# menickname/waafle

Hardware: AMD Instinct MI355X
Metric: contigs scored/sec + k2 clade-pair evals/sec at 1/2/4/8 MI355X vs CPU ref (higher is better)
Workload: dtype f64

## Files before the change

### waafle_amd/csrc/wf_device.h

```cpp
#pragma once
#include "wf_internal.h"

#include "waafle_hip.h"
#include "wf_lanes.h"

namespace wf {

namespace {


constexpr uint64_t kKeyPad = ~0ull;

#include "wf_stamps.h"
constexpr int kLocVirtual = 0xFFFF;

__device__ __forceinline__ void note_ppot(const KArgs& K, int c, int iteration, int Pp) {
  if (!K.ppot || Pp < 2) return;
  const uint64_t old = (uint64_t)K.ppot[c];
  if (iteration > (int)(old >> 40))
    K.ppot[c] = (int64_t)(((uint64_t)iteration << 40) | ((old & ((1ull << 40) - 1ull)) + (uint64_t)Pp));
}

__device__ __forceinline__ bool e2_no_option(const KArgs& K, int c, int iteration, int64_t pair_evals, bool root,
                                             int32_t* pend) {
// ... 90 lines not shown
    int a = __shfl_up(x, d, 64), b = __shfl_up(y, d, 64);
    if (lane >= d) { x += a; y += b; }
  }
  if (lane == 63) { ctl.red_i[w] = x; ctl.red_j[w] = y; }
  __syncthreads();
  int b1 = 0, b2 = 0, s1 = 0, s2 = 0;
#pragma unroll
  for (int i = 0; i < NT / 64; ++i) {
    int a = ctl.red_i[i], b = ctl.red_j[i];
    if (i < w) { b1 += a; b2 += b; }
    s1 += a;
    s2 += b;
  }
  __syncthreads();
  *p1 = b1 + x - v1;
  *p2 = b2 + y - v2;
  *t1 = s1;
  *t2 = s2;
}

__device__ __forceinline__ bool better(double r2, long long k2, double r, long long k) {
  return k2 >= 0 && (k < 0 || r2 > r || (r2 == r && k2 > k));
}

template <int NT>
__device__ __forceinline__ void block_argmax(double& r, long long& k, Ctl& ctl) {
#pragma unroll
  for (int off = 32; off > 0; off >>= 1) {
    double r2 = __shfl_xor(r, off, 64);
    long long k2 = __shfl_xor(k, off, 64);
    if (better(r2, k2, r, k)) { r = r2; k = k2; }
  }
  if (lane_id() == 0) { ctl.red_r[wave_id()] = r; ctl.red_k[wave_id()] = k; }
  __syncthreads();
  if (threadIdx.x == 0) {
    double br = ctl.red_r[0];
    long long bk = ctl.red_k[0];
    for (int i = 1; i < NT / 64; ++i)
      if (better(ctl.red_r[i], ctl.red_k[i], br, bk)) { br = ctl.red_r[i]; bk = ctl.red_k[i]; }
    ctl.best_r = br;
    ctl.best_k = bk;
  }
  __syncthreads();
  r = ctl.best_r;
  k = ctl.best_k;
}

template <int NT, class T>
__device__ __forceinline__ void bitonic_sort(T* keys, int n) {
  for (int k = 2; k <= n; k <<= 1) {
    for (int j = k >> 1; j > 0; j >>= 1) {
      for (int i = threadIdx.x; i < n; i += NT) {
        int ixj = i ^ j;
        if (ixj > i) {
          T a = keys[i], b = keys[ixj];
          bool up = (i & k) == 0;
          if ((a > b) == up) { keys[i] = b; keys[ixj] = a; }
        }
      }
      __syncthreads();
    }
  }
}


__device__ __forceinline__ int lca2(const KArgs& K, int a, int b) {
  if (a < 0) return b;
  if (b < 0) return a;
  if (a == b) return a;
  if (K.lin) {
    const int4* ra = reinterpret_cast<const int4*>(K.lin + (int64_t)a * kLin);
    const int4* rb = reinterpret_cast<const int4*>(K.lin + (int64_t)b * kLin);
    int4 x[kLin / 4], y[kLin / 4];
#pragma unroll
    for (int i = 0; i < kLin / 4; ++i) { x[i] = ra[i]; y[i] = rb[i]; }
    int r = x[0].x;
#pragma unroll
    for (int i = 0; i < kLin / 4; ++i) {
      if (x[i].x >= 0 && x[i].x == y[i].x) r = x[i].x;
      if (x[i].y >= 0 && x[i].y == y[i].y) r = x[i].y;
      if (x[i].z >= 0 && x[i].z == y[i].z) r = x[i].z;
      if (x[i].w >= 0 && x[i].w == y[i].w) r = x[i].w;
    }
    return r;
  }
  int da = K.depth[a], db = K.depth[b];
  while (da > db) { a = K.parent[a]; --da; }
  while (db > da) { b = K.parent[b]; --db; }
  while (a != b) { a = K.parent[a]; b = K.parent[b]; }
  return a;
}

__device__ __forceinline__ int block_lca(const KArgs& K, const int* list, int m, Ctl& ctl) {
  if (m <= 0) return -1;
  if (m == 1) return list[0];
  if (wave_id() == 0) {
    int acc = -1;
    for (int i = lane_id(); i < m; i += 64) acc = lca2(K, acc, list[i]);
#pragma unroll
    for (int off = 32; off > 0; off >>= 1) {
      int o = __shfl_xor(acc, off, 64);
      acc = lca2(K, acc, o);
    }
    if (lane_id() == 0) ctl.lca_out = acc;
  }
  __syncthreads();
  int r = ctl.lca_out;
  __syncthreads();
  return r;
}


constexpr int kMaxDepth = 7;
constexpr int kGroupMax = 64;

__device__ int gen_leaves(int off0, int cl, int4* out, int8_t* sched = nullptr, int stride = 0) {
  int so[8], sl[8], ss[8], sf[8];
#pragma unroll
  for (int i = 0; i < 8; ++i) { so[i] = 0; sl[i] = 0; ss[i] = 0; sf[i] = 0; }
  int cnt = 0;
  auto push = [&](int o, int l) {
#pragma unroll
    for (int i = 7; i > 0; --i) { so[i] = so[i - 1]; sl[i] = sl[i - 1]; ss[i] = ss[i - 1]; sf[i] = sf[i - 1]; }
    so[0] = o; sl[0] = l; ss[0] = 0; sf[0] = cnt;
  };
  auto pop = [&]() {
#pragma unroll
    for (int i = 0; i < 7; ++i) { so[i] = so[i + 1]; sl[i] = sl[i + 1]; ss[i] = ss[i + 1]; sf[i] = sf[i + 1]; }
  };
  int sp = 1;
  so[0] = off0; sl[0] = cl; ss[0] = 0; sf[0] = 0;
  while (sp > 0) {
    if (sl[0] > kLeafMax && ss[0] == 0) {
      int h = sl[0] / 2;
      h -= h % 8;
      ss[0] = 1;
      push(so[0], h);
      ++sp;
      continue;
    }
    const int lo = so[0], ll = sl[0];
    int adds = 0;
    pop();
    --sp;
    ++cnt;
    while (sp > 0) {
      if (ss[0] == 1) {
        int h = sl[0] / 2;
        h -= h % 8;
        ss[0] = 2;
        if (sched && sp - 1 < kMaxDepth && sf[0] < stride)
          sched[sf[0] * 8 + (sp - 1)] = (int8_t)cnt;
        push(so[0] + h, sl[0] - h);
        ++sp;
        break;
      }
      ++adds;
      pop();
      --sp;
    }
    if (out) out[cnt - 1] = make_int4(lo, ll, adds, 0);
  }
  return cnt;
}

__device__ int leaves_of_length(int n) {
  int cnt = 0;
  for (int o = 0; o < n; o += kNpyBuf) cnt += gen_leaves(o, min(kNpyBuf, n - o), nullptr);
  return cnt;
}

template <class F>
__device__ double serial_block(int o, int l, F f) {
  if (l < 8) {
    double r = 0.0;
    for (int i = 0; i < l; ++i) r += f(o + i);
    return r;
  }
  double r0 = f(o), r1 = f(o + 1), r2 = f(o + 2), r3 = f(o + 3);
  double r4 = f(o + 4), r5 = f(o + 5), r6 = f(o + 6), r7 = f(o + 7);
  int i = 8;
  const int m = l - (l & 7);
  for (; i < m; i += 8) {
    r0 += f(o + i); r1 += f(o + i + 1); r2 += f(o + i + 2); r3 += f(o + i + 3);
    r4 += f(o + i + 4); r5 += f(o + i + 5); r6 += f(o + i + 6); r7 += f(o + i + 7);
  }
  double res = ((r0 + r1) + (r2 + r3)) + ((r4 + r5) + (r6 + r7));
  for (; i < l; ++i) res += f(o + i);
  return res;
}

template <class F>
__device__ double serial_pairwise(int off0, int cl, F f) {
  if (cl <= kLeafMax) return serial_block(off0, cl, f);
  int so[8], sl[8], ss[8];
#pragma unroll
  for (int i = 0; i < 8; ++i) { so[i] = 0; sl[i] = 0; ss[i] = 0; }
  auto push = [&](int o, int l) {
#pragma unroll
    for (int i = 7; i > 0; --i) { so[i] = so[i - 1]; sl[i] = sl[i - 1]; ss[i] = ss[i - 1]; }
    so[0] = o; sl[0] = l; ss[0] = 0;
  };
  auto pop = [&]() {
#pragma unroll
    for (int i = 0; i < 7; ++i) { so[i] = so[i + 1]; sl[i] = sl[i + 1]; ss[i] = ss[i + 1]; }
  };
  double a0 = 0.0, a1 = 0.0, a2 = 0.0, a3 = 0.0, a4 = 0.0, a5 = 0.0, a6 = 0.0, a7 = 0.0;
  int sp = 1;
  so[0] = off0; sl[0] = cl;
  while (sp > 0) {
    if (sl[0] > kLeafMax && ss[0] == 0) {
      int h = sl[0] / 2;
      h -= h % 8;
      ss[0] = 1;
      push(so[0], h);
      ++sp;
      continue;
    }
    const double v = serial_block(so[0], sl[0], f);
    a7 = a6; a6 = a5; a5 = a4; a4 = a3; a3 = a2; a2 = a1; a1 = a0; a0 = v;
    pop();
    --sp;
    while (sp > 0) {
      if (ss[0] == 1) {
        int h = sl[0] / 2;
        h -= h % 8;
        ss[0] = 2;
        push(so[0] + h, sl[0] - h);
        ++sp;
        break;
      }
      a0 = a1 + a0;
      a1 = a2; a2 = a3; a3 = a4; a4 = a5; a5 = a6; a6 = a7;
      pop();
      --sp;
    }
  }
  return a0;
}

template <class F>
__device__ __forceinline__ double np_sum(int n, F f) {
  if (n <= kLeafMax) return 0.0 + serial_block(0, n, f);
  double total = 0.0;
  for (int o = 0; o < n; o += kNpyBuf) total += serial_pairwise(o, min(kNpyBuf, n - o), f);
  return total;
}


struct Contig {
  int64_t h0, l0, mbase;
  int H, G;
  int *loc_lo, *loc_len, *loc_st, *leaf_off;
  int *loc_grp, *loc_steps, *sched_off;
  uint64_t* sched;
  int4* leaves;
  int *alo, *ahi, *ahit, *aloc, *acl;
  double* asc;
  uint64_t* maxes;
  int *ign, *um;
  uint64_t* keys;
  int *seg_start, *seg_cl, *cl_id, *pot, *mem1, *mem2, *sorder;
  double* S;
  uint64_t* mask;
  unsigned *bm1, *bm2;
  uint8_t* best_syn;
  char* xws = nullptr;
  int64_t xcap = 0;
  int* sib_of = nullptr;
  uint64_t* hm = nullptr;
};

struct SumStack {
  double s0 = 0.0, s1 = 0.0, s2 = 0.0, s3 = 0.0, s4 = 0.0, s5 = 0.0, s6 = 0.0, s7 = 0.0;
  __device__ __forceinline__ void push(double v) {
    s7 = s6; s6 = s5; s5 = s4; s4 = s3; s3 = s2; s2 = s1; s1 = s0; s0 = v;
  }
  __device__ __forceinline__ void add_top() {
    s0 = s1 + s0;
    s1 = s2; s2 = s3; s3 = s4; s4 = s5; s5 = s6; s6 = s7;
  }
};

__device__ __forceinline__ double seqsum(double v, int cnt) {
  double r = 0.0;
  for (int i = 0; i < cnt; ++i) r += v;
  return r;
}

__device__ __forceinline__ double leaf_tree(double r0, double r1, double r2, double r3, double r4,
                                            double r5, double r6, double r7) {
  return ((r0 + r1) + (r2 + r3)) + ((r4 + r5) + (r6 + r7));
}

__device__ __forceinline__ int below(int base, int bound, int m) {
  const int d = bound - base;
  return d <= 0 ? 0 : min(m, (d + 7) >> 3);
}

constexpr int kThreadLeaves = 32;
constexpr int kE2Seg = 320;
constexpr int kE2MaxG = 63;
constexpr int kPruneMax = 64;

__device__ __forceinline__ bool attaches(const DevParams& P, int qlo, int qhi, int hs, int l1,
                                         int len, int lst) {
  if (P.stranded && hs != lst) return false;
  const int l2 = l1 + len - 1;
  if (l1 > qhi || qlo > l2) return 0.0 >= P.min_overlap;
  const int ov = min(qhi, l2) - max(qlo, l1) + 1;
  const int den = min(qhi - qlo + 1, l2 - l1 + 1);
  if (ov == den) return 1.0 >= P.min_overlap;
  const double t = (double)den * P.min_overlap;
  if ((double)ov > t + fabs(t) * 1e-9) return true;
  if ((double)ov < t - fabs(t) * 1e-9) return false;
  return (double)ov / (double)den >= P.min_overlap;
}

__device__ __forceinline__ double run_leaf(int lo, int hi, double v, int st, int ln) {
  const int m = ln >> 3, be = st + (m << 3);
  hi = max(hi, lo);
  double res = 0.0;
  if (m > 0) {
    int k[8], kmin = m;
#pragma unroll
    for (int c = 0; c < 8; ++c) {
      k[c] = below(st + c, hi, m) - below(st + c, lo, m);
      kmin = min(kmin, k[c]);
    }
    double s0 = 0.0;
    for (int i = 0; i < kmin; ++i) s0 += v;
    const double s1 = s0 + v, s2 = s1 + v;
    double r[8];
#pragma unroll
    for (int c = 0; c < 8; ++c) r[c] = k[c] == kmin ? s0 : (k[c] == kmin + 1 ? s1 : s2);
    res = leaf_tree(r[0], r[1], r[2], r[3], r[4], r[5], r[6], r[7]);
  }
  for (int x = be; x < st + ln; ++x) res += (x >= lo && x < hi) ? v : 0.0;
  return res;
}

template <class F>
__device__ __forceinline__ double np_sum_seq(int n, F next) {
  if (n < 8) {
    double r = 0.0;
    for (int i = 0; i < n; ++i) r += next();
    return r;
  }
  double r0 = next(), r1 = next(), r2 = next(), r3 = next();
  double r4 = next(), r5 = next(), r6 = next(), r7 = next();
  int i = 8;
  const int m = n - (n & 7);
  for (; i < m; i += 8) {
    r0 += next(); r1 += next(); r2 += next(); r3 += next();
    r4 += next(); r5 += next(); r6 += next(); r7 += next();
  }
  double res = ((r0 + r1) + (r2 + r3)) + ((r4 + r5) + (r6 + r7));
  for (; i < n; ++i) res += next();
  return res;
}

struct PtrLut {
  const int4* p;
  __device__ __forceinline__ int4 operator()(int q) const { return p[q]; }
};
__device__ __forceinline__ uint32_t pack_leaf(int4 e) { return (uint32_t)e.x | ((uint32_t)e.y << 13) | ((uint32_t)e.z << 21); }
struct PackedLut {
  const uint32_t* p;
  __device__ __forceinline__ int4 operator()(int q) const {
    const uint32_t u = p[q];
    return make_int4((int)(u & 8191u), (int)((u >> 13) & 255u), (int)(u >> 21), 0);
  }
};

__device__ __forceinline__ double pw_const_sum(int n, double v) {
  const int a0 = n >> 4;
  int K = 0, m = n;
  unsigned sel = 0;
  while (m > 128) {
    const int a = m >> 4;
    sel |= (a != (a0 >> K) ? 1u : 0u) << K;
    m -= 8 * a;
    ++K;
  }
  int Db = 0, Dmax = -1, xB = 0, xC = 0;
  bool need16 = false;
  if (K > 0) {
    Db = max(0, 28 - __clz(a0));
    Dmax = max(K - 1, Db);
    xB = a0 >> Db;
    xC = Dmax == Db + 1 ? a0 >> (Db + 1) : 0;
    need16 = Db >= 1 && (a0 >> (Db - 1)) == 16;
  }
  const int mL = m < 8 ? m : m >> 3;
  const int imax = max(max(xB, mL), need16 ? 16 : 0);
  double t = 0.0, sB = 0.0, sC = 0.0, sL = 0.0;
  for (int i = 1; i <= imax; ++i) {
    t += v;
    sB = i == xB ? t : sB;
    sC = i == xC ? t : sC;
    sL = i == mL ? t : sL;
  }
  double R;
  if (m < 8) {
    R = sL;
  } else {
    R = 8.0 * sL;
    for (int x = 0; x < (m & 7); ++x) R += v;
  }
  double q0 = 0.0, q1 = 0.0;
  for (int d = Dmax; d >= 0; --d) {
    const int B = a0 >> d;
    if (d >= Db) {
      const double sd = d == Db ? sB : sC;
      q0 = 8.0 * sd;
      q1 = 8.0 * (sd + v);
    } else {
      const double c0 = q0, c1 = q1;
      q0 = (B & 1) ? c0 + c1 : c0 + c0;
      q1 = (B & 1) ? c1 + c1 : c0 + c1;
      if (B == 16) q0 = 8.0 * t;
    }
    if (d < K) R = (((sel >> d) & 1u) ? q1 : q0) + R;
  }
  return R;
}

struct LeafCode { int kmin, code; };
__device__ __forceinline__ LeafCode run_leaf_code(int lo, int hi, int st, int ln) {
  const int m = ln >> 3, be = st + (m << 3);
  hi = max(hi, lo);
  int k[8], kmin = m;
#pragma unroll
  for (int c = 0; c < 8; ++c) {
    k[c] = below(st + c, hi, m) - below(st + c, lo, m);
    kmin = min(kmin, k[c]);
  }
  int code = 0;
#pragma unroll
  for (int c = 0; c < 8; ++c) code |= min(k[c] - kmin, 2) << (2 * c);
  const int tail = max(0, min(st + ln, hi) - max(be, lo));
  return LeafCode{kmin, code | (tail << 16) | (m > 0 ? 1 << 20 : 0)};
}
__device__ __forceinline__ double run_leaf_value(double v, LeafCode lc, double s0) {
  double res = 0.0;
  if ((lc.code >> 20) & 1) {
    const double s1 = s0 + v, s2 = s1 + v;
    double r[8];
#pragma unroll
    for (int c = 0; c < 8; ++c) {
      const int d = (lc.code >> (2 * c)) & 3;
      r[c] = d == 0 ? s0 : (d == 1 ? s1 : s2);
    }
    res = leaf_tree(r[0], r[1], r[2], r[3], r[4], r[5], r[6], r[7]);
  }
  for (int x = (lc.code >> 16) & 15; x > 0; --x) res += v;
  return res;
}

__device__ __forceinline__ double pw_run_sum(int n, int lo, int hi, double v) {
  lo = max(lo, 0);
  hi = min(hi, n);
  if (hi <= lo) return 0.0;
  const int a0 = n >> 4;
  int K = 0, m = n;
  unsigned sel = 0;
  while (m > 128) {
    const int a = m >> 4;
    sel |= (a != (a0 >> K) ? 1u : 0u) << K;
    m -= 8 * a;
    ++K;
  }
  int Db = 0, Dmax = -1, xB = 0, xC = 0;
  bool need16 = false;
  if (K > 0) {
    Db = max(0, 28 - __clz(a0));
    Dmax = max(K - 1, Db);
    xB = a0 >> Db;
    xC = Dmax == Db + 1 ? a0 >> (Db + 1) : 0;
    need16 = Db >= 1 && (a0 >> (Db - 1)) == 16;
  }
  struct Nd { int s, z, kind, cls, t; };
  auto child = [&](const Nd& x, bool right) -> Nd {
    if (x.kind == 0) {
      const int nl = 8 * (x.z >> 4);
      return right ? Nd{x.s + nl, x.z - nl, 0, 0, x.t + 1} : Nd{x.s, nl, 1, (int)((sel >> x.t) & 1u), x.t + 1};
    }
    const int xx = x.z >> 3, xl = xx >> 1, Bt = a0 >> x.t;
    return right ? Nd{x.s + 8 * xl, 8 * (xx - xl), 1, (xx - xl) - Bt, x.t + 1} : Nd{x.s, 8 * xl, 1, xl - Bt, x.t + 1};
  };
  Nd nd{0, n, 0, 0, 0};
  int mode = 0;
  for (;;) {
    if (lo <= nd.s && hi >= nd.s + nd.z) { mode = 1; break; }
    if (nd.z <= 128) { mode = 2; break; }
    const int nl = nd.kind == 0 ? 8 * (nd.z >> 4) : 8 * ((nd.z >> 3) >> 1);
    if (hi <= nd.s + nl) nd = child(nd, false);
    else if (lo >= nd.s + nl) nd = child(nd, true);
    else break;
  }
  struct Path { int tu, ty, tc; unsigned ev, evk, evc; LeafCode lc; };
  auto walk = [&](bool suffix) -> Path {
    Path q{0, 0, 0, 0u, 0u, 0u, LeafCode{0, 0}};
    Nd x = child(nd, !suffix);
    for (;;) {
      if (suffix ? lo <= x.s : hi >= x.s + x.z) { q.tu = x.t; q.ty = x.kind; q.tc = x.cls; return q; }
      if (x.z <= 128) {
        q.tu = x.t; q.ty = 2;
        q.lc = suffix ? run_leaf_code(lo, x.s + x.z, x.s, x.z) : run_leaf_code(x.s, hi, x.s, x.z);
        return q;
      }
      const Nd L = child(x, false), R = child(x, true);
      if (suffix ? lo < R.s : hi > R.s) {
        const Nd& w = suffix ? R : L;
        q.ev |= 1u << w.t;
        q.evk |= (w.kind == 0 ? 1u : 0u) << w.t;
        q.evc |= (unsigned)w.cls << w.t;
        x = suffix ? L : R;
      } else {
        x = suffix ? R : L;
      }
    }
  };
  Path p0{0, 0, 0, 0u, 0u, 0u, LeafCode{0, 0}}, p1{0, 0, 0, 0u, 0u, 0u, LeafCode{0, 0}};
  if (mode == 0) {
    p0 = walk(true);
    p1 = walk(false);
  } else if (mode == 2) {
    p0.ty = 2;
    p0.lc = run_leaf_code(lo, hi, nd.s, nd.z);
  }
  const int k0 = p0.lc.kmin, k1 = p1.lc.kmin;
  const int mL = m < 8 ? m : m >> 3;
  const int imax = mode == 2 ? k0 : max(max(max(xB, mL), need16 ? 16 : 0), max(k0, k1));
  double t = 0.0, sB = 0.0, sC = 0.0, sL = 0.0, s0a = 0.0, s0b = 0.0;
  for (int i = 1; i <= imax; ++i) {
    t += v;
    sB = i == xB ? t : sB;
    sC = i == xC ? t : sC;
    sL = i == mL ? t : sL;
    s0a = i == k0 ? t : s0a;
    s0b = i == k1 ? t : s0b;
  }
  const double lv0 = p0.ty == 2 ? run_leaf_value(v, p0.lc, s0a) : 0.0;
  if (mode == 2) return lv0;
  const double lv1 = p1.ty == 2 ? run_leaf_value(v, p1.lc, s0b) : 0.0;
  double R;
  if (m < 8) {
    R = sL;
  } else {
    R = 8.0 * sL;
    for (int x = 0; x < (m & 7); ++x) R += v;
  }
  double q0 = 0.0, q1 = 0.0, acc0 = 0.0, acc1 = 0.0;
  for (int d = Dmax; d >= -1; --d) {
    const int u = d + 1;
    if (d >= 0) {
      const int B = a0 >> d;
      if (d >= Db) {
        const double sd = d == Db ? sB : sC;
        q0 = 8.0 * sd;
        q1 = 8.0 * (sd + v);
      } else {
        const double c0 = q0, c1 = q1;
        q0 = (B & 1) ? c0 + c1 : c0 + c0;
        q1 = (B & 1) ? c1 + c1 : c0 + c1;
        if (B == 16) q0 = 8.0 * t;
      }
    }
    if (mode == 1) {
      if (u == nd.t) return nd.kind == 0 ? R : (nd.cls ? q1 : q0);
    } else {
      if (u == p0.tu) acc0 = p0.ty == 2 ? lv0 : (p0.ty == 0 ? R : (p0.tc ? q1 : q0));
      if (u <= p0.tu && ((p0.ev >> u) & 1u))
        acc0 = acc0 + (((p0.evk >> u) & 1u) ? R : (((p0.evc >> u) & 1u) ? q1 : q0));
      if (u == p1.tu) acc1 = p1.ty == 2 ? lv1 : (p1.ty == 0 ? R : (p1.tc ? q1 : q0));
      if (u <= p1.tu && ((p1.ev >> u) & 1u))
        acc1 = (((p1.evc >> u) & 1u) ? q1 : q0) + acc1;
      if (u == nd.t + 1) return acc0 + acc1;
    }
    if (d >= 0 && d < K) R = (((sel >> d) & 1u) ? q1 : q0) + R;
  }
  return 0.0;
}

template <class LT>
__device__ __forceinline__ double one_run_mean(LT lt, int nl, int len, int lo, int hi, double v) {
  hi = max(hi, lo);
  if (lo <= 0 && hi >= len && len < kNpyBuf)
    return (0.0 + pw_const_sum(len, v)) / (double)len;
  if (len < kNpyBuf)
    return (0.0 + pw_run_sum(len, lo, hi, v)) / (double)len;
  int pst0 = -1, pln0 = 0, pst1 = -1, pln1 = 0;
  int L0 = -1, L1 = -1, L2 = -1, L3 = -1;
#pragma unroll 4
  for (int q = 0; q < nl; ++q) {
    const int4 e = lt(q);
    const int le = e.x + e.y;
    const bool in = lo <= e.x && le <= hi && lo < hi;
    const bool out = le <= lo || e.x >= hi || lo >= hi;
    if (!in && !out) {
      if (pst0 < 0) { pst0 = e.x; pln0 = e.y; } else { pst1 = e.x; pln1 = e.y; }
    } else if (in && e.y != L0 && e.y != L1 && e.y != L2 && e.y != L3) {
      if (L0 < 0) L0 = e.y; else if (L1 < 0) L1 = e.y; else if (L2 < 0) L2 = e.y; else L3 = e.y;
    }
  }
// ... 1085 lines not shown
```

### waafle_amd/csrc/wf_fast.hip

```cpp
#include <algorithm>
#include <cstdlib>

#include "wf_device.h"
#include "wf_lanes.h"

namespace wf {

namespace {

constexpr int kSlotBits = 9;
constexpr int kCladeShift = 15;
constexpr uint32_t kSlotMask = (1u << kSlotBits) - 1;
constexpr int kLoc0 = 64;
constexpr int kLut0 = 256;
constexpr int kAnn0 = 64;
constexpr int kRuns0 = 64;
constexpr int kMultiAtt0 = 32;
constexpr int kRunsL0 = 32;
constexpr int kMultiAttL0 = 16;
constexpr int kXcds = 8;
constexpr int kRollWaves = 4;
constexpr int kPot0 = 64;
constexpr int kS0 = 640;

// ... 421 lines not shown
  double br = -__builtin_inf();
  long long bk = -1;
  for (int i = 0; i + 1 < Pp; ++i) {
    const uint64_t mi = pmask[i];
    for (int j = i + 1 + lane; j < Pp; j += 64) {
      if ((mi | pmask[j]) != full) continue;
      const double r = pair_rank(C, i, j, Gu);
      const long long key = (long long)i * Pp + j;
      if (better(r, key, br, bk)) { br = r; bk = key; }
    }
  }
  each_stride([&](auto J) {
    const double r2 = xor_lanes<decltype(J)::value>(br);
    const long long k2 = xor_lanes<decltype(J)::value>(bk);
    if (better(r2, k2, br, bk)) { br = r2; bk = k2; }
  });
  if (bk >= 0) {
    const int bi = (int)(bk / Pp), bj = (int)(bk % Pp);
    int b_ok = 0, b_dir = 0, b_c1p = 0, b_c2p = 0;
    double bcrit = 0.0;
    if (lane == 0) {
      const OptEval e = eval_two_call(K, C, Pn, bi, bj, nullptr, F.best_syn());
      b_ok = e.ok; b_dir = e.dir; b_c1p = e.c1p; b_c2p = e.c2p;
      bcrit = pair_crit(C, bi, bj, Gu);
    }
    b_ok = lane_bcast(b_ok, 0); b_dir = lane_bcast(b_dir, 0);
    b_c1p = lane_bcast(b_c1p, 0); b_c2p = lane_bcast(b_c2p, 0);
    bcrit = lane_bcast(bcrit, 0);
    wave_sync();
    int n_in = 0;
    bool all_ok = true, all_same = true;
    uint64_t b1 = 0, b2 = 0;
    for (int i = 0; i + 1 < Pp; ++i) {
      const uint64_t mi = pmask[i];
      for (int j = i + 1 + lane; j < Pp; j += 64) {
        if ((mi | pmask[j]) != full) continue;
        const double r = pair_rank(C, i, j, Gu);
        if (!((br - r) <= P.range)) continue;
        const OptEval e = eval_two_call(K, C, Pn, i, j, F.best_syn(), nullptr);
        ++n_in;
        all_ok = all_ok && e.ok;
        all_same = all_same && e.same;
        b1 |= 1ull << e.c1p;
        b2 |= 1ull << e.c2p;
      }
    }
    n_in = wave_sum_dpp(n_in);
    b1 = wave_or_dpp(b1);
    b2 = wave_or_dpp(b2);
    all_ok = __ballot(!all_ok) == 0ull;
    all_same = __ballot(!all_same) == 0ull;
    int kind;
    if (n_in == 0) kind = (P.dis2 == 0) ? 3 : (P.dis2 == 1 ? 0 : 4);
    else if (n_in == 1 || P.dis2 == 0) kind = 1;
    else if (P.dis2 == 1) kind = 0;
    else kind = (all_ok && all_same) ? 2 : 0;
    if (kind == 4) {
      if (lane == 0) K.status[c] = WF_E_BADINPUT;
      return kDecDone;
    }
    bool have_ok = false;
    int lca1 = -1, lca2v = -1;
    const int m1 = __popcll(b1), m2 = __popcll(b2);
    if (kind == 2) {
      const bool in1 = lane < Pp && ((b1 >> lane) & 1ull), in2 = lane < Pp && ((b2 >> lane) & 1ull);
      lca1 = wave_lca(K, in1 ? F.cl()[lane] : -1);
      lca2v = wave_lca(K, in2 ? F.cl()[lane] : -1);
      bool keep = true;
      if (!P.allow_lca) {
        const int nl = lca2(K, lca1, lca2v);
        keep = !(nl == lca1 || nl == lca2v);
      }
      have_ok = keep;
      if (have_ok) {
        if (in1) K.meld[C.mbase + __popcll(b1 & lanes_below())] = F.cl()[lane];
        if (in2) K.meld[C.mbase + m1 + __popcll(b2 & lanes_below())] = F.cl()[lane];
      }
    } else if (kind == 1) {
      have_ok = b_ok != 0;
    } else if (kind == 3) {
      have_ok = true;
    }
    if (have_ok) {
      if (lane < G) K.syn[l0 + lane] = F.best_syn()[lane];
      if (lane == 0) {
        K.call[c] = WF_CALL_LGT;
        K.crit[c] = bcrit;
        K.rank[c] = br;
        K.dir[c] = (int8_t)b_dir;
        K.c1[c] = (kind == 2) ? lca1 : F.cl()[b_c1p];
        K.c2[c] = (kind == 2) ? lca2v : F.cl()[b_c2p];
        K.nm1[c] = (kind == 2) ? m1 : 0;
        K.nm2[c] = (kind == 2) ? m2 : 0;
        K.iters[c] = (int16_t)iteration;
        K.pair_evals[c] = pair_evals;
      }
      return kDecDone;
    }
  }
  return (Pn == 0 || root) ? kDecStop : kDecRaise;
}

template <int CAP, bool FULL, bool ROLL = false>
__global__ __launch_bounds__(64, FULL ? 2 : (ROLL ? kRollWaves : 4)) void k_wave(const SArgs S_arg, int64_t* ccnt, int64_t* cleaves, int32_t* pend,
                                             const int32_t* list, int n_list, const int64_t* n_dev, int rollup,
                                             int start_level_arg) {
  static_assert(!(FULL && ROLL), "the roll-up passes are first-form launches");
  const int start_level = ROLL ? start_level_arg : 0;
  if (n_dev) n_list = (int)*n_dev;
  if (S_arg.wq && (int)blockIdx.x >= n_list) return;
  extern __shared__ __attribute__((aligned(16))) char smem[];
  WaveSmem<CAP, FULL>& F = *reinterpret_cast<WaveSmem<CAP, FULL>*>(smem);
  const int lane = threadIdx.x;
  const bool xmap = gridDim.x % kXcds == 0;
  const int xb = (int)gridDim.x / kXcds, xj = (int)blockIdx.x / kXcds, xx = (int)blockIdx.x % kXcds;
  for (int it = 0;; ++it) {
    int ci;
    if (S_arg.wq) {
      unsigned long long q = 0;
      if (lane == 0) q = atomicAdd(S_arg.wq, 1ull);
      ci = __builtin_amdgcn_readfirstlane((int)q);
    } else {
      ci = xmap ? (it * kXcds + xx) * xb + xj : (int)blockIdx.x + it * (int)gridDim.x;
    }
    if (ci >= n_list) break;
    const int c = list ? list[ci] : ci;
    WLAP_MARK();
    const SArgs& S = kernarg_fresh<SArgs>(S_arg);
    const KArgs& K = S.k;
    const DevParams& P = K.p;
    const int nsys = K.n_sys;
    const bool ann_on = !ROLL && nsys > 0;
    if (FULL && P.weak == 2) continue;
    const int64_t h0 = K.hit_off[c], h1 = K.hit_off[c + 1];
    constexpr int kHB = 4;
    int r_qlo[kHB], r_qhi[kHB], r_hs[kHB], r_cl[kHB];
    double r_scv[kHB], r_sc[kHB];
    uint32_t r_m[kHB];
    auto load_round = [&](int64_t hq) {
#pragma unroll
      for (int b = 0; b < kHB; ++b) {
        const int64_t h = hq + 64 * b + lane;
        r_qlo[b] = 0; r_qhi[b] = 0; r_hs[b] = 0; r_cl[b] = 0;
        r_scv[b] = 0.0; r_sc[b] = 0.0; r_m[b] = 0u;
        if (h < h1) {
          r_scv[b] = K.scov[h];
          r_qlo[b] = K.qlo[h];
          r_qhi[b] = K.qhi[h];
          if (P.stranded) r_hs[b] = K.hstrand[h];
          r_cl[b] = K.taxon[h];
          r_sc[b] = K.score[h];
          if (ann_on) r_m[b] = K.sysmask[h];
        }
      }
    };
    load_round(h0);
    const int64_t l0 = K.loc_off[c];
    const int G = (int)(K.loc_off[c + 1] - l0);
    const int Gs = min(G, kLoc0);
    int nl1 = 0;
    int my_lo = 0, my_hi = -1;
    if (lane < Gs) {
      const int a = K.lstart[l0 + lane], b = K.lend[l0 + lane];
      const int len = max(a, b) - min(a, b) + 1;
      my_lo = min(a, b);
      my_hi = max(a, b);
      F.lo[lane] = my_lo;
      F.len[lane] = len;
      F.st[lane] = K.lstrand[l0 + lane];
      if (len < kNpyBuf) nl1 = S.lut_off[len + 1] - S.lut_off[len];
      F.nl1[lane] = (int16_t)nl1;
    }
    const int prev_hi = __shfl_up(my_hi, 1, 64);
    const bool ordered = G <= kLoc0 && P.min_overlap > 0.0 &&
                         __ballot(lane >= 1 && lane < Gs && my_lo <= prev_hi) == 0ull;
    int lut_total;
    const int lb = wave_excl_scan(nl1, &lut_total);
    F.lbase[lane] = (int16_t)min(lb, 32767);
    const int nann = Gs * nsys;
    F.abest()[lane] = 0ull;
    F.ahit()[lane] = -1;
    const bool long_locus = __ballot(lane < Gs && F.len[lane] > 65535) != 0ull;
    bool staged = G > kLoc0 || lut_total > kLut0 || nann > kAnn0 || long_locus;
    wave_sync();
    bool lut_ready = false;
    auto load_lut = [&]() {
      for (int i = lane; i < lut_total; i += 64) {
        int g = 0;
        for (int b = 32; b > 0; b >>= 1)
          if (g + b < Gs && F.lbase[g + b] <= i) g += b;
        F.lut[i] = pack_leaf(S.lut[S.lut_off[F.len[g]] + (i - F.lbase[g])]);
      }
      wave_sync();
      lut_ready = true;
    };

    WLAP(0);
    int n_att = 0;
    long long nl_sum = 0;
    for (int64_t hq = h0; hq < h1; hq += 64 * kHB) {
      if (hq != h0) load_round(hq);
    for (int bq = 0; bq < kHB && hq + 64 * bq < h1; ++bq) {
      const int64_t hb = hq + 64 * bq;
      const int64_t h = hb + lane;
      int qlo = r_qlo[0], qhi = r_qhi[0], hs = r_hs[0], clade = r_cl[0];
      double scv = r_scv[0], sc = r_sc[0];
      uint32_t m = r_m[0];
      int n = 0;
      uint64_t am = 0ull;
#pragma unroll
      for (int b = 1; b < kHB; ++b)
        if (bq == b) {
          qlo = r_qlo[b]; qhi = r_qhi[b]; hs = r_hs[b]; clade = r_cl[b];
          scv = r_scv[b]; sc = r_sc[b]; m = r_m[b];
        }
      if (ordered && h < h1 && scv >= P.min_scov) {
        int g = 0;
#pragma unroll
        for (int k = 32; k > 0; k >>= 1) {
          const int i = min(g + k, Gs) - 1;
          if (g + k <= Gs && F.lo[i] + F.len[i] - 1 < qlo) g += k;
        }
        for (; g < Gs; ++g) {
          const int lo = F.lo[g], len = F.len[g];
          if (lo > qhi) break;
          if (attaches(P, qlo, qhi, hs, lo, len, F.st[g])) {
            ++n;
            nl_sum += len < kNpyBuf ? F.nl1[g] : leaves_for(S, len);
            am |= 1ull << g;
          }
        }
        if (ROLL && n > 0) clade = S.anc[clade];
      } else if (!ordered && h < h1 && scv >= P.min_scov) {
        for (int g = 0; g < G; ++g) {
          int lo, len, st;
          if (g < kLoc0) {
            lo = F.lo[g]; len = F.len[g]; st = F.st[g];
          } else {
            const int a = K.lstart[l0 + g], b = K.lend[l0 + g];
            lo = min(a, b); len = max(a, b) - lo + 1; st = K.lstrand[l0 + g];
          }
          if (attaches(P, qlo, qhi, hs, lo, len, st)) {
            ++n;
            nl_sum += (g < kLoc0 && len < kNpyBuf) ? F.nl1[g] : leaves_for(S, len);
            if (g < kLoc0) am |= 1ull << g;
          }
        }
        if (ROLL && n > 0) clade = S.anc[clade];
      }
      int total;
      const int o = wave_excl_scan(n, &total);
      if (!staged && n > 0 && n_att + o + n <= CAP) {
        if (!ROLL)
          for (int j = 0; j < P.jump; ++j) clade = K.parent[clade];
        const bool ann = m != 0 && sc >= P.annot_ref;
        int slot = n_att + o;
        for (uint64_t bits = am; bits; bits &= bits - 1, ++slot) {
          const int g = __builtin_ctzll(bits);
          const int len = F.len[g];
          const int h1s = max(0, qlo - F.lo[g]);
          const int h2s = min(len - 1, qhi - F.lo[g]);
          const int start = min(h1s, len);
          int stop = h2s + 1;
          if (stop < 0) { stop += len; if (stop < 0) stop = 0; }
          F.key[slot] = ((uint32_t)clade << kCladeShift) | ((uint32_t)g << kSlotBits) | (uint32_t)slot;
          F.lohi[slot] = (uint32_t)start | ((uint32_t)stop << 16);
          F.sc[slot] = sc;
          F.hit()[slot] = (int)h;
          F.sm()[slot] = (int)m;
          if (ann)
            for (int b = 0; b < nsys; ++b)
              if ((m >> b) & 1u) atomicMax(&F.abest()[g * nsys + b], dbits(sc));
        }
      }
      n_att += total;
    }
    }
    nl_sum = wave_sum_dpp(nl_sum);
    staged = staged || n_att > CAP;
    wave_sync();
    WLAP(1);
    WSTAT(16, 1);
    WSTAT(17, n_att);
    WSTAT(23, h1 - h0);
    if (!staged && G > 0 && ann_on) {
      for (int t = lane; t < n_att; t += 64) {
        const uint32_t m = (uint32_t)F.sm()[t];
        const double sc = F.sc[t];
        if (m == 0 || !(sc >= P.annot_ref)) continue;
        const int g = (int)((F.key[t] >> kSlotBits) & (kLoc0 - 1));
        const int h = F.hit()[t];
        for (int b = 0; b < nsys; ++b)
          if (((m >> b) & 1u) && F.abest()[g * nsys + b] == dbits(sc)) atomicMax(&F.ahit()[g * nsys + b], h);
      }
      wave_sync();
      if (lane < nann) K.annot[l0 * nsys + lane] = F.ahit()[lane];
    }
    WLAP(2);
    int64_t pair_evals = (ROLL && lane == 0) ? K.pair_evals[c] : 0;
    pair_evals = lane_bcast((uint64_t)pair_evals, 0);
    bool seed = false;
    bool dumped = false;
    constexpr bool kKeyOrder = !FULL && !ROLL;
    using Src = typename std::conditional<kKeyOrder, SliceSrcKey, SliceSrc>::type;
    auto slot_at = [&](int t) -> int { return kKeyOrder ? (int)(F.key[t] & kSlotMask) : t; };
    for (int level = start_level; !staged && G > 0 && h1 > h0; ++level) {
      const int iteration = level + 1;
      if (level > start_level) {
        for (int t = lane; t < n_att; t += 64) {
          const uint32_t k0 = F.key[t];
          const int parent = K.parent[(int)(k0 >> kCladeShift)];
          F.key[t] = ((uint32_t)parent << kCladeShift) | (k0 & ((1u << kCladeShift) - 1));
        }
        wave_sync();
      }
      sort_slice<(CAP + 63) / 64, !kKeyOrder>(F, n_att);
      WLAP(3);
      int ns = 0;
      for (int t0 = 0; t0 < n_att; t0 += 64) {
        const int t = t0 + lane;
        const bool head = t < n_att && (t == 0 || (F.key[t] >> kSlotBits) != (F.key[t - 1] >> kSlotBits));
        const uint64_t hm = __ballot(head);
        if (head) F.seg[ns + __popcll(hm & lanes_below())] = (F.key[t] & ~kSlotMask) | (uint32_t)t;
        ns += __popcll(hm);
      }
      if (lane == 0) F.seg[ns] = (uint32_t)n_att;
      wave_sync();
      WLAP(4);
      WSTAT(18, ns);
      double* v = F.v();
      bool fail = false;
      const bool prune = P.k1 > 0.0;
      const bool prune2 = FULL && prune && P.k2 > 0.0 && (!P.sister_on || P.sister_thr > 0.0);
      const bool prune2d = !FULL && prune && P.k2 > 0.0 && (!P.sister_on || P.sister_thr > 0.0) && P.weak != 2;
      const uint64_t allG = G >= 64 ? ~0ull : ((1ull << G) - 1ull);
      uint64_t um = 0;
      uint8_t* rc = F.rc();
      int* pp = reinterpret_cast<int*>(F.mx());
      int npp = 0;
      auto run_count = [&](int t, uint64_t mask) -> int {
        const int clade = cg_of(F, t).x;
        int cnt = 0;
        for (int q = t; q < ns; ++q) {
          const int2 cq = cg_of(F, q);
          if (cq.x != clade) break;
          cnt += (int)((mask >> cq.y) & 1ull);
        }
        return cnt;
      };
      auto sure_bits = [&]() -> uint64_t {
        uint64_t b = 0;
        for (int t = lane; t < ns; t += 64) {
          const int2 cg = cg_of(F, t);
          if (cg.x != K.unknown && v[t] >= 0.0 && v[t] >= P.kmin) b |= 1ull << cg.y;
        }
        b = wave_or_dpp(b);
        return b;
      };
      auto scan_best = [&](int t) -> double {
        const int kb = seg_first(F, t), ke = t + 1 < ns ? seg_first(F, t + 1) : n_att;
        double ub = 0.0;
        if (ke - kb == 1) {
          const int slot = slot_at(kb);
          const uint32_t x = F.lohi[slot];
          const double sc = F.sc[slot];
          const int len = F.len[cg_of(F, t).y];
          const int run = max(0, hi16(x) - lo16(x));
          return fmin(sc, sc * ((double)run / (double)len) * (1.0 + 2e-12));
        }
        for (int q = kb; q < ke; ++q) ub = fmax(ub, F.sc[slot_at(q)]);
        return ub;
      };
      auto best_score = [&](int t) -> double {
        return FULL ? scan_best(t) : -1.0 - v[t];
      };
      const double lb_thr = fmax(fmax(P.k2, P.sister_on ? P.sister_thr : 0.0), P.kmin);
      auto lb_mean = [&](int t) -> double {
        const int kb = seg_first(F, t), ke = t + 1 < ns ? seg_first(F, t + 1) : n_att;
        const double len = (double)F.len[cg_of(F, t).y];
        double lb = 0.0;
        for (int q = kb; q < ke; ++q) {
          const int slot = slot_at(q);
          const uint32_t x = F.lohi[slot];
          const int run = max(0, hi16(x) - lo16(x));
          lb = fmax(lb, F.sc[slot] * ((double)run / len) * (1.0 - 2e-12));
        }
        return lb;
      };
      auto lb_sure = [&](int t) -> bool { return lb_mean(t) >= lb_thr; };
      const bool lb_um = !FULL && prune2d && S.wave_two && S.dump_cap > 0 && G <= kE2MaxG &&
                         ns <= kE2Seg && P.weak == 0 && P.kmin > 0.0;
      auto lb_um_bits = [&](uint64_t open_) -> uint64_t {
        uint64_t b = 0;
        for (int t = lane; t < ns; t += 64) {
          const int2 cg = cg_of(F, t);
          if (cg.x != K.unknown && ((open_ >> cg.y) & 1ull) && v[t] < 0.0 && -1.0 - v[t] >= P.kmin &&
              lb_mean(t) >= P.kmin * (1.0 + 1e-12))
            b |= 1ull << cg.y;
        }
        return wave_or_dpp(b);
      };
      int n_pass0 = -1;
      if (prune) {
        constexpr int kCh = (CAP + 63) / 64;
        uint64_t hd[kCh];
#pragma unroll
        for (int i = 0; i < kCh; ++i) {
          const int t = 64 * i + lane;
          hd[i] = __ballot(t < ns && (t == 0 || (F.seg[t - 1] >> kCladeShift) != (F.seg[t] >> kCladeShift)));
        }
        const uint64_t le = lane == 63 ? ~0ull : (2ull << lane) - 1ull;
        int rs[kCh];
        int carry = 0;
#pragma unroll
        for (int i = 0; i < kCh; ++i) {
          const uint64_t m = hd[i] & le;
          rs[i] = m ? 64 * i + 63 - __clzll(m) : carry;
          carry = hd[i] ? 64 * i + 63 - __clzll(hd[i]) : carry;
        }
        carry = ns;
        int rsz[kCh];
#pragma unroll
        for (int i = kCh - 1; i >= 0; --i) {
          const int t = 64 * i + lane;
          const uint64_t m = hd[i] & ~le;
          const int re = m ? 64 * i + __ffsll((unsigned long long)m) - 1 : carry;
          carry = hd[i] ? 64 * i + __ffsll((unsigned long long)hd[i]) - 1 : carry;
          rsz[i] = re - rs[i];
          if (t < ns) {
            v[t] = FULL ? -1.0 : -1.0 - scan_best(t);
            rc[t] = (uint8_t)rsz[i];
          }
        }
        uint16_t* lst = F.list();
        n_pass0 = 0;
#pragma unroll
        for (int i = 0; i < kCh; ++i) {
          const int t = 64 * i + lane;
          const bool in = t < ns && rsz[i] == G;
          const uint64_t im = __ballot(in);
          if (in) lst[n_pass0 + __popcll(im & lanes_below())] = (uint16_t)t;
          n_pass0 += __popcll(im);
        }
        wave_sync();
      }
      const double bound = P.kmin * (1.0 - 1e-12), bound2 = P.k2 * (1.0 - 1e-12);
      const double bound_s = P.sister_thr * (1.0 - 1e-12);
      uint64_t open = 0;
      int outcome = 0;
      bool compact_ok = false;
      int e2_np = 0;
      bool e2_pairs = false;
      bool dump = false;
      const bool can_dump = !FULL && S.dump_cap > 0;
      WLAP(5);
      for (int pass = prune ? 0 : 3;;) {
        WLAP(8);
        WSTAT(19, 1);
        WSTAT(24 + pass, 1);
        int n = ns;
        const uint16_t* list = nullptr;
        if (pass == 1) {
          F.mx()[lane] = 0ull;
          wave_sync();
          for (int t = lane; t < ns; t += 64) {
            const int2 cg = cg_of(F, t);
            if (v[t] < 0.0 && cg.x != K.unknown && ((open >> cg.y) & 1ull))
              atomicMax(&F.mx()[cg.y], dbits(best_score(t)));
          }
          wave_sync();
        }
        if (pass == 0 && n_pass0 >= 0) {
          n = n_pass0;
          list = F.list();
        } else if (pass != 3) {
          uint16_t* lst = F.list();
          const int gu = __popcll(um);
          n = 0;
          for (int t0 = 0; t0 < ns; t0 += 64) {
            const int t = t0 + lane;
            bool in = false;
            if (t < ns) {
              const int2 cg = cg_of(F, t);
              if (pass == 0) {
                in = (int)rc[t] == G;
              } else if (pass == 1 || pass == 7) {
                in = v[t] < 0.0 && cg.x != K.unknown && ((open >> cg.y) & 1ull) && best_score(t) >= bound;
                if (pass == 1 && in) {
                  const double ub = best_score(t);
                  in = false;
                  const unsigned long long want = ((unsigned long long)dbits(ub) << 0);
                  in = F.mx()[cg.y] == want;
                }
              } else if (pass == 2) {
                in = v[t] < 0.0 && ((um >> cg.y) & 1ull) && (int)rc[t] == gu;
              } else if (pass == 4) {
                in = v[t] < 0.0 && best_score(t) >= bound2;
                if (!FULL && in && lb_sure(t)) {
                  in = false;
                  rc[t] |= 0x80;
                }
              } else if (pass == 5) {
                if (v[t] < 0.0) {
                  in = (rc[t] & 3) == 1;
                  if (!in && P.sister_on && best_score(t) >= bound_s) {
                    const int sp = K.sibp[cg.x];
                    for (int i = 0; i < npp && !in; ++i) in = pp[i] == sp;
                  }
                }
              } else {
                in = v[t] < 0.0;
              }
            }
            const uint64_t im = __ballot(in);
            if (in) lst[n + __popcll(im & lanes_below())] = (uint16_t)t;
            n += __popcll(im);
          }
          wave_sync();
          list = lst;
        }
        WLAP(6);
        WSTAT(20, n);
        WSTAT(40 + pass, n);
        for (int s0 = 0; s0 < n; s0 += 64) {
          const int s = s0 + lane < n ? (list ? (int)list[s0 + lane] : s0 + lane) : ns;
          bool multi = false, big = false;
          int g = 0, len = 0, nl = 0;
          bool one_run = false;
          int lo = 0, hi = 0;
          double vv = 0.0;
          if (s < ns) {
            const int kb = seg_first(F, s), ke = s + 1 < ns ? seg_first(F, s + 1) : n_att, na = ke - kb;
            g = cg_of(F, s).y;
            len = F.len[g];
            nl = F.nl1[g];
            const bool thread_ok = len < kNpyBuf && nl <= kThreadLeaves;
            if (na == 1) {
              if (thread_ok) {
                const int slot = slot_at(kb);
                lo = lo16(F.lohi[slot]); hi = hi16(F.lohi[slot]); vv = F.sc[slot];
                one_run = true;
              }
            } else if (na <= kPruneMax) {
              double Fw = 0.0;
              for (int t = kb; t < ke; ++t) {
                const int slot = slot_at(t);
                const uint32_t x = F.lohi[slot];
                const double sc = F.sc[slot];
                if (lo16(x) <= 0 && hi16(x) >= len && sc > Fw) Fw = sc;
              }
              int kept = 0;
              for (int t = kb; t < ke; ++t) {
                const int slot = slot_at(t);
                const uint32_t x = F.lohi[slot];
                kept += (lo16(x) < hi16(x) && F.sc[slot] > Fw) ? 1 : 0;
              }
              if (kept == 0 && thread_ok) { lo = 0; hi = len; vv = Fw; one_run = true; }
            }
            if (one_run) {
            } else if ((FULL || ROLL || na <= kMultiAttL0) && nl <= 64 && len < kNpyBuf) {
              multi = true;
              big = na > (FULL ? kMultiAtt0 : kMultiAttL0);
            }
            else
              fail = true;
          }
          if (!lut_ready && __ballot(multi) != 0ull) load_lut();
          WLAP(15);
          if (one_run) v[s] = one_run_mean(PackedLut{F.lut + F.lbase[g]}, nl, len, lo, hi, vv);
          WLAP(pass == 0 ? 7 : (pass == 6 ? 11 : 14));
          uint64_t mlist = __ballot(multi);
          constexpr bool kFlat = ROLL;
          if constexpr (kFlat) {
            if (mlist != 0ull) {
              int kb = 0, ke = 0;
              if (multi) { kb = seg_first(F, s); ke = s + 1 < ns ? seg_first(F, s + 1) : n_att; }
              const double m = flat_leaf_means(Src{F.key, F.lohi, F.sc}, F.lut + F.lbase[multi ? g : 0], mlist,
                                               kb, ke, nl, len, F.runs());
              if (multi) v[s] = m;
            }
            mlist = 0;
          } else if ((FULL || ROLL) && (__popcll(mlist) >= 3 || __ballot(big) != 0ull)) {
            if (multi) {
              const int kb = seg_first(F, s), ke = s + 1 < ns ? seg_first(F, s + 1) : n_att;
              v[s] = lane_seg_mean(Src{F.key, F.lohi, F.sc}, kb, ke, PackedLut{F.lut + F.lbase[g]}, nl, len);
            }
            mlist = 0;
          }
          if constexpr (!kFlat)
          for (uint64_t mm = mlist; mm; mm &= mm - 1) {
            const int src = __builtin_ctzll(mm);
            const int s2 = lane_bcast(s, src);
            const int kb = seg_first(F, s2), na = (s2 + 1 < ns ? seg_first(F, s2 + 1) : n_att) - kb;
            const int g2 = lane_bcast(g, src), len2 = lane_bcast(len, src), nl2 = lane_bcast(nl, src);
            int lo = 0, hi = 0;
            double sc = 0.0;
            if (lane < na) {
              const int slot = slot_at(kb + lane);
              const uint32_t x = F.lohi[slot];
              if (lo16(x) < hi16(x)) { lo = lo16(x); hi = hi16(x); sc = F.sc[slot]; }
            }
            const double mean = wave_seg_mean(PackedLut{F.lut + F.lbase[g2]}, nl2, len2, lo, hi, sc, F.runs());
            if (lane == 0) v[s2] = mean;
          }
          WLAP(pass == 0 ? 12 : 13);
        }
        wave_sync();
        WLAP(7);
        bool e1_now = false;
        if (pass == 0) {
          if (P.weak != 0 || P.kmin <= 0.0) {
            um = allG;
            e1_now = true;
          } else {
            um = sure_bits();
            open = allG & ~um;
            if (open && lb_um) {
              um |= lb_um_bits(open);
              open = allG & ~um;
            }
            if (open) { pass = 1; continue; }
            e1_now = true;
          }
        } else if (pass == 1 || pass == 7) {
          um |= sure_bits();
          if (pass == 1 && (open & ~um)) {
            open &= ~um;
            pass = 7;
            continue;
          }
          if (um != allG && um != 0ull) {
            for (int t = lane; t < ns; t += 64)
              if (t == 0 || cg_of(F, t - 1).x != cg_of(F, t).x) {
                const int cnt = run_count(t, ~0ull), cu = run_count(t, um);
                for (int q = t; q < t + cnt; ++q) rc[q] = (uint8_t)cu;
              }
            wave_sync();
            pass = 2;
            continue;
          }
          e1_now = true;
        } else if (pass == 2) {
          e1_now = true;
        } else if (pass == 3) {
          F.mx()[lane] = 0ull;
          wave_sync();
          for (int t = lane; t < ns; t += 64) {
            const int2 cg = cg_of(F, t);
            const double x = v[t];
            if (cg.x != K.unknown && x > 0.0) atomicMax(&F.mx()[cg.y], dbits(x));
          }
          wave_sync();
          const double mxl = __longlong_as_double((long long)F.mx()[lane]);
          um = __ballot(lane < G && (P.weak != 0 || mxl >= P.kmin));
          e1_now = true;
        } else if (pass == 4) {
          const bool members = !FULL;
          int ph = -1, pcnt = 0, np0 = 0;
          uint64_t pm = 0;
          for (int t0 = 0; t0 < ns; t0 += 64) {
            const int t = t0 + lane;
            const bool head = t < ns && (t == 0 || cg_of(F, t - 1).x != cg_of(F, t).x);
            bool pot = false;
            uint64_t m = 0;
            int cnt = 0;
            if (head) {
              const int clade = cg_of(F, t).x;
              for (int q = t; q < ns; ++q) {
                const int2 cq = cg_of(F, q);
                if (cq.x != clade) break;
                ++cnt;
                if (v[q] >= P.k2 || (rc[q] & 0x80)) { pot = true; m |= 1ull << cq.y; }
              }
              for (int q = t; q < t + cnt; ++q) rc[q] = (uint8_t)((rc[q] & 0x80) | (pot ? 1 : 0));
            }
            m &= um;
            const uint64_t im = __ballot(head && pot);
            if (members)
              for (uint64_t r = im; r; r &= r - 1) {
                const int src = __builtin_ctzll(r);
                const int dst = np0 + __popcll(im & ((1ull << src) - 1ull));
                const int hs = lane_bcast(t, src), hc = lane_bcast(cnt, src);
                const uint64_t ms = lane_bcast(m, src);
                if (lane == dst) { ph = hs; pcnt = hc; pm = ms; }
              }
            np0 += __popcll(im);
          }
          wave_sync();
          if (members && np0 <= 64) {
            bool member = false;
            for (int j = 0; j < np0; ++j) {
              const uint64_t mj = lane_bcast(pm, j);
              member = member || (lane != j && (pm | mj) == um);
            }
            if (lane < np0 && !member)
              for (int q = ph; q < ph + pcnt; ++q) rc[q] = (uint8_t)((rc[q] & 0x80) | 2);
            wave_sync();
            e2_np = np0;
            e2_pairs = __ballot(lane < np0 && member) != 0ull;
          }
          npp = 0;
          int npot = 0;
          for (int t0 = 0; t0 < ns; t0 += 64) {
            const int t = t0 + lane;
            const bool in = t < ns && (rc[t] & 3) && (t == 0 || cg_of(F, t - 1).x != cg_of(F, t).x);
            const uint64_t im = __ballot(in);
            const bool mem_in = in && (rc[t] & 3) == 1;
            const uint64_t mm = __ballot(mem_in);
            if (mem_in && npp + __popcll(mm & lanes_below()) < 64)
              pp[npp + __popcll(mm & lanes_below())] = K.parent[cg_of(F, t).x];
            npp = min(npp + __popcll(mm), 64);
            npot += __popcll(im);
          }
          wave_sync();
          pass = (!FULL && npot > 64) ? 6 : 5;
          compact_ok = pass == 5;
          continue;
        } else {
          break;
        }
        if (!e1_now) break;
        WLAP(32);
        if (__ballot(fail) != 0ull) { staged = __ballot(fail) != 0ull; outcome = 2; break; }
        const int Gu = __popcll(um);
        if (Gu == 0) {
          if (level > 0 && lane == 0) {
            K.iters[c] = (int16_t)min(iteration, 32767);
            K.pair_evals[c] = pair_evals;
            K.status[c] = WF_E_EMPTYMASK;
          }
          outcome = 2;
          break;
        }
          double br = -__builtin_inf(), bcrit = 0.0;
          long long bk = -1;
          double* rank = F.rank();
          auto option_rank = [&](int t, double& crit) -> double {
            const int clade = cg_of(F, t).x;
            if ((t == 0 || cg_of(F, t - 1).x != clade) && (!prune || (int)rc[t] == Gu) &&
                !(P.weak == 2 && clade == K.unknown)) {
              double rnk;
              sparse_score(F, v, t, ns, clade, um, Gu, crit, rnk);
// ... 308 lines not shown
```

Baseline: 112.9 million.

## Tighten clade score bounds with coverage envelope integral and prune candidate groups

In the ROLL variant, the per-segment score upper bound is now the coverage-weighted envelope integral of hit scores over the gene length, replacing the plain maximum score. The same value then serves as a tight lower bound through marker_lb. A new interval pre-pass computes the best lower-bound group mean and drops full-width candidate groups whose upper bound cannot come within P.range of it, shrinking the list passed to the pairwise evaluation. The cost is an O(len-segments × hits) envelope sweep per segment plus extra wave syncs, and the tolerances used in pruning could misclassify borderline groups.

```diff
diff --git a/waafle_amd/csrc/wf_device.h b/waafle_amd/csrc/wf_device.h
--- a/waafle_amd/csrc/wf_device.h
+++ b/waafle_amd/csrc/wf_device.h
@@ -416,6 +416,39 @@
 constexpr int kE2Seg = 320;
 constexpr int kE2MaxG = 63;
 constexpr int kPruneMax = 64;
+
+constexpr double kEnvSlack = 2e-12;
+template <class Rg, class Sc>
+__device__ __forceinline__ double env_integral(Rg range, Sc score, int kb, int ke, int len, double& best) {
+  double acc = 0.0;
+  best = 0.0;
+  for (int p = 0; p < len;) {
+    int nx = len;
+    double val = 0.0;
+    for (int q = kb; q < ke; ++q) {
+      int l, h;
+      range(q, l, h);
+      if (l >= h) continue;
+      if (l <= p && p < h) {
+        const double s = score(q);
+        val = s > val ? s : val;
+        nx = h < nx ? h : nx;
+      } else if (l > p) {
+        nx = l < nx ? l : nx;
+      }
+    }
+    best = val > best ? val : best;
+    acc += val * (double)(nx - p);
+    p = nx;
+  }
+  return acc / (double)len;
+}
+__device__ __forceinline__ double marker_ub(double v) { return -1.0 - v; }
+__device__ __forceinline__ double marker_lb(double v) {
+  const double ub = -1.0 - v;
+  const double lb = ub * (1.0 - 5e-12) - 4.5e-16 * (1.0 + ub);
+  return lb > 0.0 ? lb : 0.0;
+}
 
 __device__ __forceinline__ bool attaches(const DevParams& P, int qlo, int qhi, int hs, int l1,
                                          int len, int lst) {
diff --git a/waafle_amd/csrc/wf_fast.hip b/waafle_amd/csrc/wf_fast.hip
--- a/waafle_amd/csrc/wf_fast.hip
+++ b/waafle_amd/csrc/wf_fast.hip
@@ -747,6 +747,8 @@
     bool seed = false;
     bool dumped = false;
     constexpr bool kKeyOrder = !FULL && !ROLL;
+    constexpr bool kEnvOn = ROLL;
+    constexpr bool kIvOn = ROLL;
     using Src = typename std::conditional<kKeyOrder, SliceSrcKey, SliceSrc>::type;
     auto slot_at = [&](int t) -> int { return kKeyOrder ? (int)(F.key[t] & kSlotMask) : t; };
     for (int level = start_level; !staged && G > 0 && h1 > h0; ++level) {
@@ -813,6 +815,17 @@
           const int run = max(0, hi16(x) - lo16(x));
           return fmin(sc, sc * ((double)run / (double)len) * (1.0 + 2e-12));
         }
+        if (kEnvOn && ke - kb <= kPruneMax) {
+          double best;
+          const double I = env_integral(
+              [&](int q, int& l, int& h) {
+                const uint32_t x = F.lohi[slot_at(q)];
+                l = lo16(x); h = hi16(x);
+              },
+              [&](int q) -> double { return F.sc[slot_at(q)]; },
+              kb, ke, F.len[cg_of(F, t).y], best);
+          return fmin(best * (1.0 + 1e-14), I * (1.0 + kEnvSlack));
+        }
         for (int q = kb; q < ke; ++q) ub = fmax(ub, F.sc[slot_at(q)]);
         return ub;
       };
@@ -822,6 +835,7 @@
       const double lb_thr = fmax(fmax(P.k2, P.sister_on ? P.sister_thr : 0.0), P.kmin);
       auto lb_mean = [&](int t) -> double {
         const int kb = seg_first(F, t), ke = t + 1 < ns ? seg_first(F, t + 1) : n_att;
+        if (kEnvOn && ke - kb <= kPruneMax) return marker_lb(v[t]);
         const double len = (double)F.len[cg_of(F, t).y];
         double lb = 0.0;
         for (int q = kb; q < ke; ++q) {
@@ -877,12 +891,51 @@
             rc[t] = (uint8_t)rsz[i];
           }
         }
+        if (kIvOn) wave_sync();
+        if (kIvOn && lb_um && P.range >= 0.0 && lb_um_bits(allG) == allG) {
+          double best_lb = -__builtin_inf();
+#pragma unroll 1
+          for (int t0 = 0; t0 < ns; t0 += 64) {
+            const int t = t0 + lane;
+            const bool head = t < ns && (int)rc[t] == G &&
+                              (t == 0 || (F.seg[t - 1] >> kCladeShift) != (F.seg[t] >> kCladeShift));
+            if (head) {
+              double cl = __builtin_inf(), sl = 0.0;
+              for (int q = t; q < t + G; ++q) {
+                const double l = lb_mean(q);
+                cl = fmin(cl, l);
+                sl += l;
+              }
+              if (cl >= P.k1 * (1.0 + 1e-12)) best_lb = fmax(best_lb, sl / (double)G * (1.0 - 1e-12));
+            }
+          }
+          best_lb = wave_butterfly(best_lb, [](double a, double b) { return b > a ? b : a; });
+          const double need = (best_lb - P.range) - 1e-11 * (1.0 + fabs(best_lb) + P.range);
+#pragma unroll 1
+          for (int t0 = 0; t0 < ns; t0 += 64) {
+            const int t = t0 + lane;
+            const bool head = t < ns && (int)rc[t] == G &&
+                              (t == 0 || (F.seg[t - 1] >> kCladeShift) != (F.seg[t] >> kCladeShift));
+            if (head) {
+              double cu = __builtin_inf(), su = 0.0;
+              for (int q = t; q < t + G; ++q) {
+                const double u = marker_ub(v[q]);
+                cu = fmin(cu, u);
+                su += u;
+              }
+              const bool keep = cu >= P.k1 * (1.0 - 1e-12) && su / (double)G * (1.0 + 1e-12) >= need;
+              if (!keep)
+                for (int q = t; q < t + G; ++q) rc[q] = 0;
+            }
+          }
+          wave_sync();
+        }
         uint16_t* lst = F.list();
         n_pass0 = 0;
 #pragma unroll
         for (int i = 0; i < kCh; ++i) {
           const int t = 64 * i + lane;
-          const bool in = t < ns && rsz[i] == G;
+          const bool in = t < ns && (kIvOn ? (int)rc[t] : rsz[i]) == G;
           const uint64_t im = __ballot(in);
           if (in) lst[n_pass0 + __popcll(im & lanes_below())] = (uint16_t)t;
           n_pass0 += __popcll(im);
```

Measured after the change: 116.9 million, median of 6. 1.04x the previous value.
